# lionelblonde/sac-td3-cudagraphs-pytorch

Measured on NVIDIA B200. Metric: gradient updates/sec (batch 256, Hopper shapes), higher is better.
Workload: dtype f32

## Files before the change

### sac_td3_cudagraphs_pytorch_b200/csrc/api.cu

```cuda
#include <cstdarg>
#include <cstdio>
#include <cstdlib>
#include <cstring>

#include "common.cuh"

namespace b2rl {
cudaError_t launch_critic_fused(const b2rl_update_args_t&, cudaStream_t);
cudaError_t launch_actor_fused(const b2rl_update_args_t&, cudaStream_t);
cudaError_t launch_alpha(const b2rl_update_args_t&, float, cudaStream_t);
cudaError_t launch_alpha_adam(float*, uint64_t*, int, float, const b2rl_agent_hp_t*, float, float*, cudaStream_t);
cudaError_t launch_predict(const b2rl_update_args_t&, const float*, int, int, float, uint64_t, float*, cudaStream_t);
cudaError_t launch_wgrad(const b2rl_update_args_t&, int, int, const b2rl_adam_args_t*, cudaStream_t, int skip_vec = 0);
cudaError_t launch_adam(const b2rl_adam_args_t&, cudaStream_t);
cudaError_t launch_sumsq(const float*, int64_t, int64_t, int64_t, int64_t, int, float*, float*, cudaStream_t);
cudaError_t launch_bump(uint64_t*, int, int, cudaStream_t);
cudaError_t launch_gather(const float*, int64_t, int64_t, b2rl_rowfmt_t, int, int, const int64_t*, int64_t*, float*,
                          uint64_t, uint64_t*, int, int, int, cudaStream_t);
cudaError_t launch_extend(float*, int64_t, int64_t, b2rl_rowfmt_t, const float*, int, cudaStream_t);
cudaError_t launch_publish(const float*, int, float*, uint64_t*, uint64_t*, cudaStream_t);
cudaError_t launch_extend_dev(float*, int64_t, int64_t, b2rl_rowfmt_t, const float*, int, int, uint64_t*, cudaStream_t);
int max_in_dim_critic();
int max_in_dim_actor();
cudaError_t init_critic();
// ... 332 lines not shown
                      "wide_critic_scalars");
}
int b2rl_wide_actor_loss(const float* q0, const float* q1, const float* logp, const float* log_alpha, int32_t td3, int32_t M,
                         float* dzq0, float* dzq1, float* part, const b2rl_stack_t* stack, void* stream) {
  if (int rc = check_stack(stack, "wide_actor_loss")) return rc;
  if (!q0 || !dzq0 || !part || M < 1 || (!td3 && (!q1 || !dzq1 || !logp || !log_alpha)))
    return fail(B2RL_E_INVALID, "wide_actor_loss: bad arguments");
  return check_launch(b2rl::launch_wide_actor_loss(q0, q1, logp, log_alpha, td3, M, dzq0, dzq1, part, make_stk(stack), (cudaStream_t)stream), "wide_actor_loss");
}
int b2rl_wide_dqda(const float* dz1, const float* w1a, int32_t A, int32_t M, float* dqda, const b2rl_stack_t* stack, void* stream) {
  if (int rc = check_stack(stack, "wide_dqda")) return rc;
  if (!dz1 || !w1a || !dqda || A < 1 || A > 32 || M < 1) return fail(B2RL_E_INVALID, "wide_dqda: bad arguments");
  return check_launch(b2rl::launch_wide_dqda(dz1, w1a, A, M, dqda, make_stk(stack), (cudaStream_t)stream), "wide_dqda");
}
int b2rl_wide_actor_head_bwd(const float* dqda0, const float* dqda1, const float* save, const float* min_ac,
                             const float* max_ac, const float* log_alpha, int32_t td3, int32_t A, int32_t M, float* du,
                             float* part_du, const b2rl_stack_t* stack, void* stream) {
  if (int rc = check_stack(stack, "wide_actor_head_bwd")) return rc;
  if (!dqda0 || !save || !min_ac || !max_ac || !du || !part_du || A < 1 || A > 32 || M < 1 || (!td3 && !log_alpha))
    return fail(B2RL_E_INVALID, "wide_actor_head_bwd: bad arguments");
  return check_launch(b2rl::launch_wide_actor_head_bwd(dqda0, dqda1, save, min_ac, max_ac, log_alpha, td3, A, M, du, part_du,
                                                       make_stk(stack), (cudaStream_t)stream), "wide_actor_head_bwd");
}
int b2rl_wide_actor_scalars(const float* part_s, const float* part_du, int32_t P, int32_t M, int32_t out_dim, int32_t td3,
                            const float* log_alpha, float* G, int64_t off_b3, float* out, const b2rl_stack_t* stack, void* stream) {
  if (int rc = check_stack(stack, "wide_actor_scalars")) return rc;
  if (!part_s || !part_du || !G || !out || P < 1 || M < 1 || out_dim < 1 || out_dim > B2RL_MAX_OUT)
    return fail(B2RL_E_INVALID, "wide_actor_scalars: bad arguments");
  return check_launch(b2rl::launch_wide_actor_scalars(part_s, part_du, P, M, out_dim, td3, log_alpha, G, off_b3, out, make_stk(stack), (cudaStream_t)stream),
                      "wide_actor_scalars");
}
int b2rl_wide_alpha_grad(const float* logp2, int32_t M, float targ_ent, float* alpha_state, const b2rl_stack_t* stack, void* stream) {
  if (int rc = check_stack(stack, "wide_alpha_grad")) return rc;
  if (!logp2 || !alpha_state || M < 1) return fail(B2RL_E_INVALID, "wide_alpha_grad: bad arguments");
  return check_launch(b2rl::launch_wide_alpha_grad(logp2, M, targ_ent, alpha_state, make_stk(stack), (cudaStream_t)stream), "wide_alpha_grad");
}
int64_t b2rl_tc_wgrad_scratch_floats(int32_t MA, int32_t Bn, int32_t n_agents) {
  if (MA < 1 || Bn < 1 || n_agents < 0) return -1;
  const int64_t per_agent = (int64_t)b2rl::tc_wgrad_splits(Bn, MA, n_agents > 0) * ((MA + 127) / 128 * 128) * B2RL_HID;
  return per_agent * (n_agents > 0 ? n_agents : 1);
}
int b2rl_tc_wgrad(const float* A, int64_t lda, int32_t a_cols, int32_t MA, const float* Bm, int32_t Bn, float* C, float* Ct,
                  float* scratch, int32_t x3, uint64_t* bump, const b2rl_stack_t* stack, void* stream) {
  if (int rc = check_stack(stack, "tc_wgrad")) return rc;
  if (!A || !Bm || !C || !scratch || MA < 1 || a_cols < MA || lda < a_cols || (lda & 3) || Bn < 1)
    return fail(B2RL_E_INVALID, "tc_wgrad: bad arguments");
  if (!aligned16(A) || !aligned16(Bm) || !aligned16(C) || !aligned16(scratch)) return fail(B2RL_E_INVALID, "tc_wgrad: 16-byte aligned tensors");
  if (Ct && (MA & 3)) return fail(B2RL_E_INVALID, "tc_wgrad: the transposed copy needs MA % 4 == 0");
  return check_launch(b2rl::launch_tc_wgrad(A, lda, a_cols, MA, Bm, Bn, C, Ct, scratch, x3, (unsigned long long*)bump, make_stk(stack),
                                            stack != nullptr, (cudaStream_t)stream), "tc_wgrad");
}
int b2rl_wgrad(const b2rl_update_args_t* a, int32_t actor_step, int32_t bump_counter, int32_t skip_vectors, void* stream) {
  if (int rc = check_update(a, actor_step != 0)) return rc;
  if (bump_counter < -1 || bump_counter > 3) return fail(B2RL_E_INVALID, "wgrad: bad bump_counter");
  return check_launch(b2rl::launch_wgrad(*a, actor_step != 0, bump_counter, nullptr, (cudaStream_t)stream, skip_vectors != 0), "wgrad");
}

int b2rl_publish_logs(const float* out, int32_t n_agents, float* host_out, uint64_t* seq_dev, uint64_t* host_seq,
                      void* stream) {
  if (!out || !host_out || !seq_dev || !host_seq || n_agents < 1) return fail(B2RL_E_INVALID, "publish_logs: bad arguments");
  return check_launch(b2rl::launch_publish(out, n_agents, host_out, seq_dev, host_seq, (cudaStream_t)stream), "publish_logs");
}

static int check_opt(const b2rl_update_args_t* a, const b2rl_adam_args_t* o, int64_t begin, int64_t end, int counter) {
  if (!o) return B2RL_OK;
  if (o->n_seg < 1 || o->n_seg > B2RL_MAX_SEG) return fail(B2RL_E_INVALID, "opt: n_seg %d out of range", o->n_seg);
  if (o->lo)
    return fail(B2RL_E_INVALID, "opt: the fused optimizer does not keep a lo mirror current; use the three-launch form");
  if (a->agent_hp || o->agent_hp)
    return fail(B2RL_E_INVALID, "opt: the fused optimizer takes no per-agent hyperparameter table; use the three-launch form");
  const b2rl_seg_t& s0 = o->seg[0];
  if (!s0.do_adam || s0.clip || s0.grad_scale != 1.0f || s0.begin != begin || s0.end != end || s0.counter != counter)
    return fail(B2RL_E_INVALID, "opt: seg[0] must be an unclipped, unscaled Adam segment over the trained nets");
  for (int i = 1; i < o->n_seg; ++i) {
    const b2rl_seg_t& s = o->seg[i];
    if (s.do_adam || !s.do_polyak || s.begin < 0 || s.end < s.begin || (s.begin & 3) || (s.end & 3) || s.end > a->region_stride)
      return fail(B2RL_E_INVALID, "opt: extra segment %d must be a 4-float aligned Polyak-only span", i);
  }
  return B2RL_OK;
}

static int critic_update(const b2rl_update_args_t* a, int td3, const b2rl_adam_args_t* opt, void* stream) {
  if (int rc = check_update(a, false)) return rc;
  if (opt && a->new_rows) return fail(B2RL_E_INVALID, "new_rows is not supported by the fused-optimizer entry point");
  if (int rc = check_opt(a, opt, a->critic[0].begin, a->critic[1].end, B2RL_CTR_Q)) return rc;
  if ((a->hp.td3 != 0) != (td3 != 0)) return fail(B2RL_E_INVALID, "hp.td3 does not match the entry point");
  if (int rc = check_launch(b2rl::launch_critic_fused(*a, (cudaStream_t)stream), "critic_fused")) return rc;
  return check_launch(b2rl::launch_wgrad(*a, 0, B2RL_CTR_Q, opt, (cudaStream_t)stream), "critic wgrad");
}
int b2rl_critic_update_sac(const b2rl_update_args_t* a, void* stream) { return critic_update(a, 0, nullptr, stream); }
int b2rl_critic_update_td3(const b2rl_update_args_t* a, void* stream) { return critic_update(a, 1, nullptr, stream); }
int b2rl_critic_update_opt(const b2rl_update_args_t* a, const b2rl_adam_args_t* opt, void* stream) {
  if (!a || !opt) return fail(B2RL_E_INVALID, "null args");
  return critic_update(a, a->hp.td3 != 0, opt, stream);
}

static int actor_update(const b2rl_update_args_t* a, int td3, const b2rl_adam_args_t* opt, void* stream) {
  if (int rc = check_update(a, true)) return rc;
  if (int rc = check_opt(a, opt, a->actor.begin, a->actor.end, B2RL_CTR_PI)) return rc;
  if ((a->hp.td3 != 0) != (td3 != 0)) return fail(B2RL_E_INVALID, "hp.td3 does not match the entry point");
  if (int rc = check_launch(b2rl::launch_actor_fused(*a, (cudaStream_t)stream), "actor_fused")) return rc;
  return check_launch(b2rl::launch_wgrad(*a, 1, B2RL_CTR_PI, opt, (cudaStream_t)stream), "actor wgrad");
}
int b2rl_actor_update_sac(const b2rl_update_args_t* a, void* stream) { return actor_update(a, 0, nullptr, stream); }
int b2rl_actor_update_td3(const b2rl_update_args_t* a, void* stream) { return actor_update(a, 1, nullptr, stream); }
int b2rl_actor_update_opt(const b2rl_update_args_t* a, const b2rl_adam_args_t* opt, void* stream) {
  if (!a || !opt) return fail(B2RL_E_INVALID, "null args");
  return actor_update(a, a->hp.td3 != 0, opt, stream);
}

int b2rl_alpha_update(const b2rl_update_args_t* a, float log_alpha_lr, void* stream) {
  if (int rc = check_update(a, false)) return rc;
  if (a->hp.td3) return fail(B2RL_E_INVALID, "alpha_update is SAC-only");
  if (!(log_alpha_lr >= 0.f)) return fail(B2RL_E_INVALID, "log_alpha_lr must be >= 0");
  return check_launch(b2rl::launch_alpha(*a, log_alpha_lr, (cudaStream_t)stream), "alpha_update");
}

int b2rl_alpha_adam(float* log_alpha, uint64_t* counters, int32_t n_agents, float log_alpha_lr, float grad_scale,
                    float* out, void* stream) {
  if (!log_alpha || !counters || n_agents < 1 || !(log_alpha_lr > 0.f))
    return fail(B2RL_E_INVALID, "alpha_adam: bad arguments");
  return check_launch(b2rl::launch_alpha_adam(log_alpha, counters, n_agents, log_alpha_lr, nullptr, grad_scale, out,
                                              (cudaStream_t)stream),
                      "alpha_adam");
}

int b2rl_alpha_adam_hp(float* log_alpha, uint64_t* counters, int32_t n_agents, const b2rl_agent_hp_t* hp, float grad_scale,
                       float* out, void* stream) {
  if (!log_alpha || !counters || n_agents < 1 || !hp) return fail(B2RL_E_INVALID, "alpha_adam_hp: bad arguments");
  if (int rc = check_hp(hp, "alpha_adam_hp")) return rc;
  return check_launch(b2rl::launch_alpha_adam(log_alpha, counters, n_agents, 0.f, hp, grad_scale, out, (cudaStream_t)stream),
                      "alpha_adam_hp");
}

int b2rl_grad_sumsq(const float* arena, int64_t region_stride, int64_t arena_agent_stride, int64_t begin, int64_t end,
                    int32_t n_agents, float* sumsq, float* scratch, void* stream) {
  if (!arena || !sumsq || !scratch || begin < 0 || end < begin || n_agents < 1)
    return fail(B2RL_E_INVALID, "grad_sumsq: bad arguments");
  return check_launch(b2rl::launch_sumsq(arena, region_stride, arena_agent_stride, begin, end, n_agents, sumsq, scratch,
                                         (cudaStream_t)stream),
                      "grad_sumsq");
}

int b2rl_adam_polyak_multi(const b2rl_adam_args_t* a, void* stream) {
  if (!a || !a->arena || !a->counters) return fail(B2RL_E_INVALID, "adam: null args");
  if (a->n_seg < 1 || a->n_seg > B2RL_MAX_SEG) return fail(B2RL_E_INVALID, "adam: n_seg %d out of range", a->n_seg);
  if (a->n_agents < 1 || a->n_agents > 65535) return fail(B2RL_E_INVALID, "adam: bad n_agents");
  if (!aligned16(a->arena) || (a->region_stride & 3) || (a->arena_agent_stride & 3))
    return fail(B2RL_E_INVALID, "adam: arena must be 16-byte aligned, strides multiples of 4 floats");
  if (a->lo && (!aligned16(a->lo) || (a->lo_agent_stride & 3) || a->lo_agent_stride < 2 * a->region_stride))
    return fail(B2RL_E_INVALID, "adam: the lo mirror must be 16-byte aligned, its agent stride >= 2 regions and a multiple of 4 floats");
  if (a->n_shadow < 0 || a->n_shadow > 3) return fail(B2RL_E_INVALID, "adam: n_shadow %d out of range", a->n_shadow);
  if (int rc = check_hp(a->agent_hp, "adam")) return rc;
  for (int q = 0; q < a->n_shadow; ++q) {
    const int64_t src = a->shadow_src[q], dst = a->shadow_dst[q], n = (int64_t)B2RL_HID * B2RL_HID;
    if (src < 0 || dst < 0 || (src & 3) || (dst & 3) || src + n > a->region_stride || dst + n > a->region_stride ||
        (src < dst + n && dst < src + n))
      return fail(B2RL_E_INVALID, "adam: shadow pair %d must be two disjoint, 4-float aligned 256x256 spans of a region", q);
    for (int i = 0; i < a->n_seg; ++i) {
      const b2rl_seg_t& s = a->seg[i];
      const bool in_src = src >= s.begin && src + n <= s.end, in_dst = dst >= s.begin && dst + n <= s.end;
      const bool cut = (src < s.end && src + n > s.begin && !in_src) || (dst < s.end && dst + n > s.begin && !in_dst);
      if (cut || in_src != in_dst) return fail(B2RL_E_INVALID, "adam: segment %d splits shadow pair %d", i, q);
    }
  }
  for (int i = 0; i < a->n_seg; ++i) {
    const b2rl_seg_t& s = a->seg[i];
// ... 56 lines not shown
```

### sac_td3_cudagraphs_pytorch_b200/csrc/wgrad.cu

```cuda
#include "adam_math.cuh"

namespace b2rl {

constexpr int TM = 32, TN = 32;
constexpr int WT = 256, WW = WT / 32;

struct GemmJob {
  const float* A;
  const float* Bm;
  float* C;
  float* Ct;
  int lda, ldb, M;
};

struct OptCtx {
  int adam, polyak;
  AdamScalars k;
  float beta2, omb1, omb2, eps, pk;
  int64_t region;
};
static __device__ __noinline__ void opt_apply4(const OptCtx* ocp, float* gptr) {
  const OptCtx& oc = *ocp;
  float* P = gptr - 4 * oc.region;
  float4 p = *reinterpret_cast<const float4*>(P);
  float4 tg = make_float4(0.f, 0.f, 0.f, 0.f);
  if (oc.polyak) tg = *reinterpret_cast<const float4*>(P + oc.region);
  if (oc.adam) {
    const float4 g = *reinterpret_cast<const float4*>(gptr);
    float4 m = *reinterpret_cast<const float4*>(P + 2 * oc.region);
    float4 v = *reinterpret_cast<const float4*>(P + 3 * oc.region);
    adam_elem(p.x, g.x, m.x, v.x, oc.k, oc.beta2, oc.omb1, oc.omb2, oc.eps);
    adam_elem(p.y, g.y, m.y, v.y, oc.k, oc.beta2, oc.omb1, oc.omb2, oc.eps);
    adam_elem(p.z, g.z, m.z, v.z, oc.k, oc.beta2, oc.omb1, oc.omb2, oc.eps);
    adam_elem(p.w, g.w, m.w, v.w, oc.k, oc.beta2, oc.omb1, oc.omb2, oc.eps);
    *reinterpret_cast<float4*>(P) = p;
    *reinterpret_cast<float4*>(P + 2 * oc.region) = m;
    *reinterpret_cast<float4*>(P + 3 * oc.region) = v;
  }
  if (oc.polyak) {
    tg.x = polyak_elem(tg.x, p.x, oc.pk); tg.y = polyak_elem(tg.y, p.y, oc.pk);
    tg.z = polyak_elem(tg.z, p.z, oc.pk); tg.w = polyak_elem(tg.w, p.w, oc.pk);
    *reinterpret_cast<float4*>(P + oc.region) = tg;
  }
}
static __device__ __noinline__ void opt_apply1(const OptCtx* ocp, float* gptr) {
  const OptCtx& oc = *ocp;
  float* P = gptr - 4 * oc.region;
  float p = *P;
  float tg = oc.polyak ? P[oc.region] : 0.f;
  if (oc.adam) {
    float m = P[2 * oc.region], v = P[3 * oc.region];
    adam_elem(p, *gptr, m, v, oc.k, oc.beta2, oc.omb1, oc.omb2, oc.eps);
    *P = p; P[2 * oc.region] = m; P[3 * oc.region] = v;
  }
  if (oc.polyak) P[oc.region] = polyak_elem(tg, p, oc.pk);
}

constexpr int CHUNK = 32;
struct WgradSmem {
  union {
    float stage[WW][2][CHUNK][TM];
    float red[WW][TM][TN + 1];
  };
};

__device__ __forceinline__ void cp_async16(void* smem_dst, const void* gsrc, bool valid) {
  const unsigned d = (unsigned)__cvta_generic_to_shared(smem_dst);
  const int n = valid ? 16 : 0;
  asm volatile("cp.async.cg.shared.global [%0], [%1], 16, %2;" ::"r"(d), "l"(gsrc), "r"(n) : "memory");
}

template <typename Setup>
__device__ void gemm_tile(const GemmJob& J, int B, int m0, int n0, WgradSmem& S, const OptCtx* oc, Setup setup) {
  const int t = threadIdx.x, w = t >> 5, l = t & 31;
  const int mi = (l >> 2) * 4, ni = (l & 3) * 8;
  const int bs = (B + WW - 1) / WW;
  const int bA = min(B, w * bs), bB = min(B, bA + bs);
  float acc[4][8];
#pragma unroll
  for (int i = 0; i < 4; ++i)
#pragma unroll
    for (int j = 0; j < 8; ++j) acc[i][j] = 0.f;
  float(*As)[TM] = S.stage[w][0];
  float(*Bs)[TM] = S.stage[w][1];
  for (int b0 = bA; b0 < bB; b0 += CHUNK) {
    const int nb = min(CHUNK, bB - b0);
    for (int idx = l; idx < nb * 8; idx += 32) {
      const int row = idx >> 3, seg = (idx & 7) * 4;
      cp_async16(&As[row][seg], J.A + (size_t)(b0 + row) * J.lda + m0 + seg, m0 + seg + 3 < J.lda);
      cp_async16(&Bs[row][seg], J.Bm + (size_t)(b0 + row) * J.ldb + n0 + seg, true);
    }
    asm volatile("cp.async.commit_group;\n cp.async.wait_group 0;" ::: "memory");
    __syncwarp();
#pragma unroll 4
    for (int row = 0; row < nb; ++row) {
      const float4 a = *reinterpret_cast<const float4*>(&As[row][mi]);
      const float4 x0 = *reinterpret_cast<const float4*>(&Bs[row][ni]);
      const float4 x1 = *reinterpret_cast<const float4*>(&Bs[row][ni + 4]);
      const float av[4] = {a.x, a.y, a.z, a.w};
      const float xv[8] = {x0.x, x0.y, x0.z, x0.w, x1.x, x1.y, x1.z, x1.w};
#pragma unroll
      for (int i = 0; i < 4; ++i)
#pragma unroll
        for (int j = 0; j < 8; ++j) acc[i][j] = fmaf(av[i], xv[j], acc[i][j]);
    }
    __syncwarp();
  }
  setup();
  __syncthreads();
#pragma unroll
  for (int i = 0; i < 4; ++i)
#pragma unroll
    for (int j = 0; j < 8; ++j) S.red[w][mi + i][ni + j] = acc[i][j];
  __syncthreads();
  const int i = t >> 3, j0 = (t & 7) * 4;
  float s[4];
#pragma unroll
  for (int j = 0; j < 4; ++j) {
    float v = S.red[0][i][j0 + j];
#pragma unroll
    for (int ww = 1; ww < WW; ++ww) v += S.red[ww][i][j0 + j];
    s[j] = v;
  }
  if (m0 + i < J.M) {
    float* gp = J.C + (size_t)(m0 + i) * HID + n0 + j0;
    const float4 g4 = make_float4(s[0], s[1], s[2], s[3]);
    *reinterpret_cast<float4*>(gp) = g4;
    if (oc) opt_apply4(oc, gp);
  }
  if (J.Ct) {
    __syncthreads();
#pragma unroll
    for (int j = 0; j < 4; ++j) S.red[0][i][j0 + j] = s[j];
    __syncthreads();
    const int jj = t >> 3, i0 = (t & 7) * 4;
    if (m0 + i0 + 3 < J.M) {
      float* gp = J.Ct + (size_t)(n0 + jj) * J.M + m0 + i0;
      const float4 g4 = make_float4(S.red[0][i0][jj], S.red[0][i0 + 1][jj], S.red[0][i0 + 2][jj], S.red[0][i0 + 3][jj]);
      *reinterpret_cast<float4*>(gp) = g4;
      if (oc) opt_apply4(oc, gp);
    }
  }
}

constexpr int XTRA_CTAS = 16;

struct WgradArgs {
  b2rl_update_args_t u;
  int actor_step;
  int bump_counter;
  int has_opt;
  int work_ctas;
  int skip_vec;
  b2rl_adam_args_t opt;
};

__device__ __forceinline__ const b2rl_net_t& net_of(const WgradArgs& W, int n) {
  return W.actor_step ? W.u.actor : W.u.critic[n];
}

__host__ __device__ inline int tiles_of_net(const b2rl_net_t& n) {
  const int nt = HID / TN;
  return ((n.in_dim + TM - 1) / TM) * nt + (HID / TM) * nt + ((n.out_dim + TM - 1) / TM) * nt;
}
constexpr int VEC_CTAS = PART_VEC + 1;

static __device__ __noinline__ unsigned long long setup_and_ticket(const WgradArgs& W, int agent, uint64_t cnt, OptCtx& oc_s) {
  uint64_t* ctr = W.u.counters + (size_t)agent * 8;
  if (W.has_opt) {
    const b2rl_seg_t& s0 = W.opt.seg[0];
    OptCtx o;
    o.adam = s0.do_adam; o.polyak = s0.do_polyak;
    o.k = adam_scalars(s0.lr, W.opt.beta1, W.opt.beta2, (float)(cnt + 1ULL));
    adam_finish(o.k, W.opt.eps);
    o.beta2 = W.opt.beta2; o.omb1 = 1.0f - W.opt.beta1; o.omb2 = 1.0f - W.opt.beta2; o.eps = W.opt.eps;
    o.pk = W.opt.polyak; o.region = W.u.region_stride;
    oc_s = o;
  }
  if (W.bump_counter < 0) return 0ULL;
  __threadfence();
  return atomicAdd((unsigned long long*)&ctr[B2RL_CTR_TICKET], 1ULL + (cnt & 0ULL));
}
template <bool OPT>
__device__ __forceinline__ void ticket_finish(const WgradArgs& W, int agent, uint64_t cnt, unsigned long long ticket) {
  if (!OPT) return;
  if (threadIdx.x != 0 || W.bump_counter < 0 || ticket != (unsigned long long)gridDim.x - 1) return;
  uint64_t* ctr = W.u.counters + (size_t)agent * 8;
  ctr[W.bump_counter] = cnt + 1ULL;
  ctr[B2RL_CTR_TICKET] = 0;
}

template <bool OPT>
__global__ void __launch_bounds__(WT) wgrad_kernel(const __grid_constant__ WgradArgs W) {
  pdl_enter();
  extern __shared__ __align__(16) unsigned char wsm_raw[];
  WgradSmem& S = *reinterpret_cast<WgradSmem*>(wsm_raw);
  __shared__ OptCtx oc_s;
  const b2rl_update_args_t& A = W.u;
  const int agent = blockIdx.y, t = threadIdx.x;
  const int B = A.batch, nblk = row_blocks(B);
  const int n_nets = W.actor_step ? 1 : 2;
  float* arena = A.arena + (size_t)agent * A.arena_agent_stride;
  float* G = arena + 4 * A.region_stride;
  const float* rows = A.rows + (size_t)agent * A.rows_agent_stride;
  float* wsb = A.workspace + (size_t)agent * A.workspace_agent_stride;
  const int nt = HID / TN;
  const OptCtx* oc = OPT ? &oc_s : nullptr;
  const int cidx = W.bump_counter >= 0 ? W.bump_counter : (W.has_opt ? W.opt.seg[0].counter : 0);
  const uint64_t cnt = (OPT && t == 0) ? A.counters[(size_t)agent * 8 + cidx] : 0ULL;
  unsigned long long ticket = 0ULL;
  auto setup = [&]() { if (OPT && t == 0) ticket = setup_and_ticket(W, agent, cnt, oc_s); };

  int id = blockIdx.x;
  if (OPT && id >= W.work_ctas) {
    const int64_t stride = (int64_t)XTRA_CTAS * WT * 4;
    float* P = arena;
    float* T = arena + A.region_stride;
    for (int si = 1; si < W.opt.n_seg; ++si) {
      const b2rl_seg_t& sg = W.opt.seg[si];
      for (int64_t i = sg.begin + ((int64_t)(id - W.work_ctas) * WT + t) * 4; i < sg.end; i += stride) {
        const float4 p = *reinterpret_cast<const float4*>(P + i);
        float4 tg = *reinterpret_cast<const float4*>(T + i);
        tg.x = polyak_elem(tg.x, p.x, W.opt.polyak); tg.y = polyak_elem(tg.y, p.y, W.opt.polyak);
        tg.z = polyak_elem(tg.z, p.z, W.opt.polyak); tg.w = polyak_elem(tg.w, p.w, W.opt.polyak);
        *reinterpret_cast<float4*>(T + i) = tg;
      }
    }
    setup();
    ticket_finish<OPT>(W, agent, cnt, ticket);
    return;
  }
  for (int n = 0; n < n_nets; ++n) {
    const b2rl_net_t& net = net_of(W, n);
    const Workspace ws = ws_carve(wsb, B, n);
    const int t1 = ((net.in_dim + TM - 1) / TM) * nt, t2 = (HID / TM) * nt, t3 = ((net.out_dim + TM - 1) / TM) * nt;
    if (id < t1 + t2 + t3) {
      GemmJob J;
      if (id < t1) {
        J = {rows, ws.dz1, G + net.w1t, nullptr, A.fmt.row_stride, HID, net.in_dim};
      } else if (id < t1 + t2) {
        id -= t1;
        J = {ws.h1, ws.dz2, G + net.w2t, net.w2n >= 0 ? G + net.w2n : nullptr, HID, HID, HID};
      } else {
        id -= t1 + t2;
        J = {ws.dz3, ws.h2, G + net.w3, nullptr, MAX_OUT, HID, net.out_dim};
      }
      gemm_tile(J, B, (id / nt) * TM, (id % nt) * TN, S, oc, setup);
      ticket_finish<OPT>(W, agent, cnt, ticket);
      return;
    }
    id -= t1 + t2 + t3;
    if (id < VEC_CTAS) {
      if (W.skip_vec) return;
      setup();
      __syncthreads();
      if (id < PART_VEC) {
        if (net.layer_norm || (id % 3) == 0) {
          const int64_t off = id == 0 ? net.b1 : id == 1 ? net.g1 : id == 2 ? net.be1 : id == 3 ? net.b2 : id == 4 ? net.g2 : net.be2;
          const float* p = ws.part + (size_t)id * HID + t;
          float s = 0.f;
#pragma unroll 16
          for (int i = 0; i < nblk; ++i) s += p[(size_t)i * PART_LEN];
          G[off + t] = s;
          if (oc) opt_apply1(oc, G + off + t);
        }
      } else {
        if (t < net.out_dim) {
          float s = 0.f;
#pragma unroll 16
          for (int i = 0; i < nblk; ++i) s += ws.part[(size_t)i * PART_LEN + PART_DB3 + t];
          G[net.b3 + t] = s;
          if (oc) opt_apply1(oc, G + net.b3 + t);
        }
        if ((t >> 5) == 2 && n == n_nets - 1) {
          const int lane = t & 31;
          float* out = A.out + (size_t)agent * 8;
          float tot = 0.f, lp = 0.f;
          for (int m = 0; m < n_nets; ++m) {
            const float* pm = ws_carve(wsb, B, m).part;
            float s0 = 0.f, s1 = 0.f;
            for (int i = lane; i < nblk; i += 32) {
              s0 += pm[(size_t)i * PART_LEN + PART_SCAL];
              s1 += pm[(size_t)i * PART_LEN + PART_SCAL + 1];
            }
            tot += warp_sum(s0) / (float)B;
            lp += warp_sum(s1);
          }
          if (lane == 0) {
            if (W.actor_step) {
              out[B2RL_OUT_ACTOR_LOSS] = tot;
              out[B2RL_OUT_LOGPI_MEAN] = lp / (float)B;
              if (!A.hp.td3) out[B2RL_OUT_ALPHA] = expf(A.log_alpha[(size_t)agent * 5]);
            } else {
              out[B2RL_OUT_QF_LOSS] = tot;
            }
          }
        }
      }
      ticket_finish<OPT>(W, agent, cnt, ticket);
      return;
    }
    id -= VEC_CTAS;
  }
  if (!OPT) {
    if (id == 0 && t == 0 && W.bump_counter >= 0) A.counters[(size_t)agent * 8 + W.bump_counter] += 1ULL;
    if (id == 0 && !W.actor_step && A.new_rows) {
      uint64_t* ctr = A.counters + (size_t)agent * 8;
      const int64_t cursor = (int64_t)ctr[B2RL_CTR_CURSOR];
      const int rs = A.fmt.row_stride, chunks = rs >> 2;
      float* sto = const_cast<float*>(A.storage) + (size_t)agent * A.storage_agent_stride;
      for (int i = t; i < A.n_new * chunks; i += blockDim.x) {
        const int r = i / chunks, c4 = i - r * chunks;
        const int64_t d = (cursor + r) % A.capacity;
        st_stream4(sto + (size_t)d * rs + 4 * c4, ld_stream4(A.new_rows + (size_t)r * rs + 4 * c4));
      }
      __syncthreads();
      if (t == 0) {
        ctr[B2RL_CTR_CURSOR] = (uint64_t)((cursor + A.n_new) % A.capacity);
        const uint64_t size = ctr[B2RL_CTR_SIZE] + (uint64_t)A.n_new;
        ctr[B2RL_CTR_SIZE] = size < (uint64_t)A.capacity ? size : (uint64_t)A.capacity;
      }
    }
    return;
  }
  setup();
  ticket_finish<OPT>(W, agent, cnt, ticket);
}

cudaError_t init_wgrad() {
  cudaError_t e = cudaFuncSetAttribute(wgrad_kernel<false>, cudaFuncAttributeMaxDynamicSharedMemorySize, (int)sizeof(WgradSmem));
  if (e == cudaSuccess)
    e = cudaFuncSetAttribute(wgrad_kernel<true>, cudaFuncAttributeMaxDynamicSharedMemorySize, (int)sizeof(WgradSmem));
  return e;
}

cudaError_t launch_wgrad(const b2rl_update_args_t& a, int actor_step, int bump_counter, const b2rl_adam_args_t* opt,
                         cudaStream_t st, int skip_vec) {
  WgradArgs W;
  W.skip_vec = skip_vec;
  W.u = a;
  W.actor_step = actor_step;
  W.bump_counter = bump_counter;
  W.has_opt = opt != nullptr;
  if (opt) W.opt = *opt;
  int ctas = 0;
  const int n_nets = actor_step ? 1 : 2;
  for (int n = 0; n < n_nets; ++n) ctas += tiles_of_net(actor_step ? a.actor : a.critic[n]) + VEC_CTAS;
  W.work_ctas = ctas;
  if (opt && opt->n_seg > 1) ctas += XTRA_CTAS;
  if (!opt) ctas += 1;
  dim3 grid(ctas, a.n_agents);
  if (opt) return launch_k(wgrad_kernel<true>, grid, dim3(WT), -1, sizeof(WgradSmem), st, W);
  return launch_k(wgrad_kernel<false>, grid, dim3(WT), -1, sizeof(WgradSmem), st, W);
}

}
```

### sac_td3_cudagraphs_pytorch_b200/engine.py

```python
from __future__ import annotations

import ctypes as C
from typing import Optional

import numpy as np
import torch

from . import _lib as L
from .agents.agent import Agent
from .replay import Batch, ReplayBuffer
from .staging import StepStaging


class LearnerEngine:
    def __init__(self, agent: Agent, rb: Optional[ReplayBuffer] = None, batch_size: Optional[int] = None,
                 use_graphs: Optional[bool] = None, record_noise: bool = False, fused_opt: bool = False,
                 fused_sample: Optional[bool] = None):
        self.agent = agent
        self.rb = rb if rb is not None else agent.rb
        assert self.rb is not None and self.rb.storage is not None, "the replay buffer must hold data"
        self.B = int(batch_size or agent.hps.batch_size)
        self.use_graphs = bool(agent.hps.cudagraphs) if use_graphs is None else use_graphs
        self.fused_opt = bool(fused_opt)
        self.fused_sample = True if fused_sample is None else bool(fused_sample)
        dev = agent.device
        self.rows = torch.zeros(self.B, agent.fmt.row_stride, dtype=torch.float32, device=dev)
        self.idx = torch.zeros(self.B, dtype=torch.int64, device=dev)
        delay = int(agent.hps.actor_update_delay)
        mk = (lambda: torch.zeros(self.B, agent.ac_dim, device=dev)) if record_noise else (lambda: None)
        self.noise_q, self.noise_pi, self.noise_alpha = mk(), [mk() for _ in range(delay)], [mk() for _ in range(delay)]
        self.args_q = agent.update_args(self.rows, eps_out=self.noise_q,
                                        storage=self.rb.storage if self.fused_sample else None, idx_out=self.idx)
        self.args_pi = [agent.update_args(self.rows, eps_out=self.noise_pi[j], eps2_out=self.noise_alpha[j])
                        for j in range(delay)]
        self.graphs: dict[tuple, torch.cuda.CUDAGraph] = {}
        self._size_on_device = -1
        self._cursor_on_device = -1
        self.launches_per_variant: dict[tuple, int] = {}
        self._stage = StepStaging(dev, (), agent.fmt.row_stride, agent.ob_dim, agent.ac_dim)
        self.host_out = self._stage.host_outs[0]
        self._keep: list = []
        self._side_stream = torch.cuda.Stream(device=dev)

    def _enqueue(self, do_actor: bool, do_polyak: bool, args_q=None, before_last_adam=None) -> int:
        ag, rb = self.agent, self.rb
        args_q = args_q or self.args_q
        st = ag._stream()
        n = 0
        if not self.fused_sample:
            L.check(ag._lib.b2rl_replay_sample_gather(
                rb.storage.data_ptr(), 0, 0, rb.fmt, self.B, 1, None, self.idx.data_ptr(), self.rows.data_ptr(),
                C.c_uint64(ag.seed), ag.counters.data_ptr(), L.CTR_Q, 0, ag.agent_id, st), "replay_sample_gather")
            n += 1
        delay = int(ag.hps.actor_update_delay) if do_actor else 0
        extra = ag.polyak_segs(critics=False, actor=True) if (ag.td3 and do_polyak and delay == 0) else []
        fused = ag.fuses_opt(self.fused_opt)
        hook = None if fused else before_last_adam
        ag.enqueue_critic_step(args_q, extra_segs=extra, polyak=do_polyak, fused_opt=fused,
                               before_adam=hook if delay == 0 else None)
        n += 2 if fused else 3
        for j in range(delay):
            ag.enqueue_actor_step(self.args_pi[j], polyak=ag.td3 and do_polyak and j == delay - 1,
                                  fused_opt=fused,
                                  before_adam=hook if (j == delay - 1 and not ag.autotune) else None)
            n += (5 if ag.hps.clip_norm > 0 else (2 if fused else 3)) + (1 if ag.autotune else 0)
        return n

    def _polyak_due(self) -> bool:
        ag = self.agent
        return ag.td3 or ((ag.qnet_updates_so_far + 1) % ag.hps.crit_targ_update_freq == 0)

    def _sync_size(self) -> None:
        if self._size_on_device != len(self.rb):
            self._size_on_device = len(self.rb)
            self.agent.counters[L.CTR_SIZE] = self._size_on_device
        if self._cursor_on_device != self.rb._cursor:
            self._cursor_on_device = self.rb._cursor
            self.agent.counters[L.CTR_CURSOR] = self._cursor_on_device

    def host_rows(self, n: int, slot: Optional[int] = None) -> torch.Tensor:
        return self._stage.rows(n, slot)

    def host_obs(self, n: int, slot: Optional[int] = None) -> torch.Tensor:
        return self._stage.obs(n, slot)

    def wait_actions(self) -> "np.ndarray":
        return self._stage.actions()

    def step_async(self, i: int, n_new: int = 0, n_obs: int = 0, explore: bool = True) -> int:
        ag, rb = self.agent, self.rb
        assert self.use_graphs, "step() is the graph path"
        slot = self._stage.begin()
        do_actor = (i % (ag.hps.actor_update_delay + 1) == 0)
        key = (do_actor, self._polyak_due(), int(n_new), slot, int(n_obs), bool(explore))
        self._sync_size()
        g = self.graphs.get(key)
        if g is None:
            g = self._capture_step(key)
        g.replay()
        if n_new:
            rb._cursor = (rb._cursor + n_new) % rb.capacity
            rb._size = min(rb.capacity, rb._size + n_new)
            self._cursor_on_device, self._size_on_device = rb._cursor, rb._size
        ag.qnet_updates_so_far += 1
        if do_actor:
            ag.actor_updates_so_far += int(ag.hps.actor_update_delay)
        return self._stage.launched(n_obs, slot)

    def wait(self, ticket: int, as_numpy: bool = False):
        return self._stage.wait(ticket, as_numpy)

    def step(self, i: int, n_new: int = 0, n_obs: int = 0, explore: bool = True) -> torch.Tensor:
        return self.wait(self.step_async(i, n_new, n_obs, explore))

    def _capture_step(self, key) -> torch.cuda.CUDAGraph:
        ag, rb, stage = self.agent, self.rb, self._stage
        do_actor, do_polyak, n_new, slot, n_obs, explore = key
        new_rows = stage.rows(n_new, slot) if n_new else None
        if n_obs:
            obs = stage.obs(n_obs, slot)
            pa = L.UpdateArgs()
            pa.hp, pa.fmt, pa.actor = ag._hyper, ag.fmt, ag.layout.actor.c_struct()
            pa.arena, pa.region_stride, pa.agent_base = ag.arena.flat.data_ptr(), ag.layout.region, ag.agent_id
            pa.min_ac, pa.max_ac, pa.counters = ag.min_ac.data_ptr(), ag.max_ac.data_ptr(), ag.counters.data_ptr()
            self._keep.append(pa)
        g = torch.cuda.CUDAGraph()
        torch.cuda.synchronize(ag.device)
        with torch.cuda.graph(g):
            n = 0
            if n_obs:
                std = float(ag.hps.actor_noise_std) if ag.td3 else 0.0
                L.check(ag._lib.b2rl_actor_predict(C.byref(pa), obs.data_ptr(), n_obs, int(explore), std,
                                                   C.c_uint64(2 ** 64 - 1), stage.device_actions(n_obs).data_ptr(), ag._stream()),
                        "actor_predict")
                stage.publish_actions(ag._lib, n_obs, slot, ag._stream())
                n += 2
            args_q = None
            if n_new and self.fused_sample and not ag.fuses_opt(self.fused_opt):
                args_q = ag.update_args(self.rows, eps_out=self.noise_q, storage=rb.storage, idx_out=self.idx,
                                        new_rows=new_rows, n_new=n_new)
                self._keep.append(args_q)
            elif n_new:
                L.check(ag._lib.b2rl_replay_extend_dev(rb.storage.data_ptr(), rb.capacity, rb.fmt,
                                                       new_rows.data_ptr(), n_new, ag.counters.data_ptr(),
                                                       ag._stream()), "replay_extend_dev")
                n += 1
            joined = []

            def publish():
                stage.publish_logs(ag._lib, ag.out, slot, ag._stream())

            def fork_publish():
                main, ev = torch.cuda.current_stream(ag.device), torch.cuda.Event()
                ev.record(main)
                self._side_stream.wait_event(ev)
                with torch.cuda.stream(self._side_stream):
                    publish()
                    done = torch.cuda.Event()
                    done.record(self._side_stream)
                joined.append(done)

            n += self._enqueue(do_actor, do_polyak, args_q, before_last_adam=fork_publish)
            if joined:
                torch.cuda.current_stream(ag.device).wait_event(joined[0])
            else:
                publish()
            n += 1
        self.launches_per_variant[key] = n
        self.graphs[key] = g
        return g

    def iteration(self, i: int) -> None:
        ag = self.agent
        do_actor = (i % (ag.hps.actor_update_delay + 1) == 0)
        key = (do_actor, self._polyak_due())
        self._sync_size()
        if not self.use_graphs:
            self.launches_per_variant[key] = self._enqueue(*key)
        else:
            g = self.graphs.get(key)
            if g is None:
                g = self._capture(key)
            g.replay()
        ag.qnet_updates_so_far += 1
        if do_actor:
            ag.actor_updates_so_far += int(ag.hps.actor_update_delay)

    def _capture(self, key) -> torch.cuda.CUDAGraph:
        g = torch.cuda.CUDAGraph()
        torch.cuda.synchronize(self.agent.device)
        with torch.cuda.graph(g):
            self.launches_per_variant[key] = self._enqueue(*key)
        self.graphs[key] = g
        return g

    def launches(self, i: int) -> int:
        key = (i % (self.agent.hps.actor_update_delay + 1) == 0, self._polyak_due())
        return self.launches_per_variant.get(key, 0)

    def logs(self) -> dict[str, torch.Tensor]:
        ag, o = self.agent, self.agent.out
        d = {"loss/qf_loss": o[L.OUT_QF_LOSS], "loss/actor_loss": o[L.OUT_ACTOR_LOSS]}
        if not ag.td3:
            d["vitals/alpha"] = o[L.OUT_ALPHA]
            if ag.autotune:
                d["loss/alpha_loss"] = o[L.OUT_ALPHA_LOSS]
        return d

    def last_batch(self) -> Batch:
        return Batch(self.rows, self.agent.fmt, self.idx)
```

Measured before the change: 16280.

## Enable fused optimizer by default and fold replay writes, prefetch, Polyak into wgrad

Makes the fused Adam/Polyak optimizer path the default when gradient clipping is off. The replay-buffer write moves into a dedicated CTA of the fused wgrad kernel, removing a separate extend launch. Optimizer state is prefetched into L1 before the GEMM tile runs, and the transposed-gradient optimizer update reuses staged shared-memory results instead of reloading state. The extra Polyak CTA count is now sized from the segment lengths, with two float4 loads per iteration. The new path adds shared-memory staging and extra synchronisation, and risks ordering problems if replay writes overlap with sampling.

```diff
diff --git a/sac_td3_cudagraphs_pytorch_b200/csrc/api.cu b/sac_td3_cudagraphs_pytorch_b200/csrc/api.cu
--- a/sac_td3_cudagraphs_pytorch_b200/csrc/api.cu
+++ b/sac_td3_cudagraphs_pytorch_b200/csrc/api.cu
@@ -438,7 +438,6 @@
 
 static int critic_update(const b2rl_update_args_t* a, int td3, const b2rl_adam_args_t* opt, void* stream) {
   if (int rc = check_update(a, false)) return rc;
-  if (opt && a->new_rows) return fail(B2RL_E_INVALID, "new_rows is not supported by the fused-optimizer entry point");
   if (int rc = check_opt(a, opt, a->critic[0].begin, a->critic[1].end, B2RL_CTR_Q)) return rc;
   if ((a->hp.td3 != 0) != (td3 != 0)) return fail(B2RL_E_INVALID, "hp.td3 does not match the entry point");
   if (int rc = check_launch(b2rl::launch_critic_fused(*a, (cudaStream_t)stream), "critic_fused")) return rc;
diff --git a/sac_td3_cudagraphs_pytorch_b200/csrc/wgrad.cu b/sac_td3_cudagraphs_pytorch_b200/csrc/wgrad.cu
--- a/sac_td3_cudagraphs_pytorch_b200/csrc/wgrad.cu
+++ b/sac_td3_cudagraphs_pytorch_b200/csrc/wgrad.cu
@@ -1,3 +1,5 @@
+#include <algorithm>
+
 #include "adam_math.cuh"
 
 namespace b2rl {
@@ -14,45 +16,56 @@
 };
 
 struct OptCtx {
-  int adam, polyak;
+  int polyak;
   AdamScalars k;
   float beta2, omb1, omb2, eps, pk;
   int64_t region;
 };
-static __device__ __noinline__ void opt_apply4(const OptCtx* ocp, float* gptr) {
+__device__ __forceinline__ void prefetch_l1(const float* p) { asm volatile("prefetch.global.L1 [%0];" ::"l"(p)); }
+__device__ __forceinline__ void opt_prefetch(const float* gptr, int64_t region, bool polyak) {
+  const float* P = gptr - 4 * region;
+  prefetch_l1(P);
+  if (polyak) prefetch_l1(P + region);
+  prefetch_l1(P + 2 * region);
+  prefetch_l1(P + 3 * region);
+}
+static __device__ __noinline__ void opt_apply4(const OptCtx* ocp, float* gptr, float4 g, float* stage) {
   const OptCtx& oc = *ocp;
   float* P = gptr - 4 * oc.region;
   float4 p = *reinterpret_cast<const float4*>(P);
   float4 tg = make_float4(0.f, 0.f, 0.f, 0.f);
   if (oc.polyak) tg = *reinterpret_cast<const float4*>(P + oc.region);
-  if (oc.adam) {
-    const float4 g = *reinterpret_cast<const float4*>(gptr);
-    float4 m = *reinterpret_cast<const float4*>(P + 2 * oc.region);
-    float4 v = *reinterpret_cast<const float4*>(P + 3 * oc.region);
-    adam_elem(p.x, g.x, m.x, v.x, oc.k, oc.beta2, oc.omb1, oc.omb2, oc.eps);
-    adam_elem(p.y, g.y, m.y, v.y, oc.k, oc.beta2, oc.omb1, oc.omb2, oc.eps);
-    adam_elem(p.z, g.z, m.z, v.z, oc.k, oc.beta2, oc.omb1, oc.omb2, oc.eps);
-    adam_elem(p.w, g.w, m.w, v.w, oc.k, oc.beta2, oc.omb1, oc.omb2, oc.eps);
-    *reinterpret_cast<float4*>(P) = p;
-    *reinterpret_cast<float4*>(P + 2 * oc.region) = m;
-    *reinterpret_cast<float4*>(P + 3 * oc.region) = v;
-  }
+  float4 m = *reinterpret_cast<const float4*>(P + 2 * oc.region);
+  float4 v = *reinterpret_cast<const float4*>(P + 3 * oc.region);
+  adam_elem(p.x, g.x, m.x, v.x, oc.k, oc.beta2, oc.omb1, oc.omb2, oc.eps);
+  adam_elem(p.y, g.y, m.y, v.y, oc.k, oc.beta2, oc.omb1, oc.omb2, oc.eps);
+  adam_elem(p.z, g.z, m.z, v.z, oc.k, oc.beta2, oc.omb1, oc.omb2, oc.eps);
+  adam_elem(p.w, g.w, m.w, v.w, oc.k, oc.beta2, oc.omb1, oc.omb2, oc.eps);
+  *reinterpret_cast<float4*>(P) = p;
+  *reinterpret_cast<float4*>(P + 2 * oc.region) = m;
+  *reinterpret_cast<float4*>(P + 3 * oc.region) = v;
   if (oc.polyak) {
     tg.x = polyak_elem(tg.x, p.x, oc.pk); tg.y = polyak_elem(tg.y, p.y, oc.pk);
     tg.z = polyak_elem(tg.z, p.z, oc.pk); tg.w = polyak_elem(tg.w, p.w, oc.pk);
     *reinterpret_cast<float4*>(P + oc.region) = tg;
   }
-}
-static __device__ __noinline__ void opt_apply1(const OptCtx* ocp, float* gptr) {
+  if (stage) {
+    constexpr int SL = TM * (TN + 1);
+    const float4 o[4] = {p, m, v, tg};
+#pragma unroll
+    for (int q = 0; q < 4; ++q) {
+      stage[q * SL] = o[q].x; stage[q * SL + 1] = o[q].y; stage[q * SL + 2] = o[q].z; stage[q * SL + 3] = o[q].w;
+    }
+  }
+}
+static __device__ __noinline__ void opt_apply1(const OptCtx* ocp, float* gptr, float g) {
   const OptCtx& oc = *ocp;
   float* P = gptr - 4 * oc.region;
-  float p = *P;
-  float tg = oc.polyak ? P[oc.region] : 0.f;
-  if (oc.adam) {
-    float m = P[2 * oc.region], v = P[3 * oc.region];
-    adam_elem(p, *gptr, m, v, oc.k, oc.beta2, oc.omb1, oc.omb2, oc.eps);
-    *P = p; P[2 * oc.region] = m; P[3 * oc.region] = v;
-  }
+  float p = P[0];
+  const float tg = oc.polyak ? P[oc.region] : 0.f;
+  float m = P[2 * oc.region], v = P[3 * oc.region];
+  adam_elem(p, g, m, v, oc.k, oc.beta2, oc.omb1, oc.omb2, oc.eps);
+  P[0] = p; P[2 * oc.region] = m; P[3 * oc.region] = v;
   if (oc.polyak) P[oc.region] = polyak_elem(tg, p, oc.pk);
 }
 
@@ -70,12 +83,17 @@
   asm volatile("cp.async.cg.shared.global [%0], [%1], 16, %2;" ::"r"(d), "l"(gsrc), "r"(n) : "memory");
 }
 
-template <typename Setup>
-__device__ void gemm_tile(const GemmJob& J, int B, int m0, int n0, WgradSmem& S, const OptCtx* oc, Setup setup) {
+template <bool OPT, typename Setup>
+__device__ void gemm_tile(const GemmJob& J, int B, int m0, int n0, WgradSmem& S, const OptCtx* oc, int64_t region, bool polyak,
+                          Setup setup) {
   const int t = threadIdx.x, w = t >> 5, l = t & 31;
   const int mi = (l >> 2) * 4, ni = (l & 3) * 8;
   const int bs = (B + WW - 1) / WW;
   const int bA = min(B, w * bs), bB = min(B, bA + bs);
+  const int i = t >> 3, j0 = (t & 7) * 4;
+  float* gp = J.C + (size_t)(m0 + i) * HID + n0 + j0;
+  const bool row_ok = m0 + i < J.M;
+  if (OPT && row_ok) opt_prefetch(gp, region, polyak);
   float acc[4][8];
 #pragma unroll
   for (int i = 0; i < 4; ++i)
@@ -113,7 +131,6 @@
 #pragma unroll
     for (int j = 0; j < 8; ++j) S.red[w][mi + i][ni + j] = acc[i][j];
   __syncthreads();
-  const int i = t >> 3, j0 = (t & 7) * 4;
   float s[4];
 #pragma unroll
   for (int j = 0; j < 4; ++j) {
@@ -122,28 +139,48 @@
     for (int ww = 1; ww < WW; ++ww) v += S.red[ww][i][j0 + j];
     s[j] = v;
   }
-  if (m0 + i < J.M) {
-    float* gp = J.C + (size_t)(m0 + i) * HID + n0 + j0;
-    const float4 g4 = make_float4(s[0], s[1], s[2], s[3]);
-    *reinterpret_cast<float4*>(gp) = g4;
-    if (oc) opt_apply4(oc, gp);
-  }
+  const float4 g4 = make_float4(s[0], s[1], s[2], s[3]);
+  if (row_ok) *reinterpret_cast<float4*>(gp) = g4;
+  if (J.Ct) __syncthreads();
+  if (OPT && row_ok) opt_apply4(oc, gp, g4, J.Ct ? &S.red[1][i][j0] : nullptr);
   if (J.Ct) {
-    __syncthreads();
 #pragma unroll
     for (int j = 0; j < 4; ++j) S.red[0][i][j0 + j] = s[j];
     __syncthreads();
     const int jj = t >> 3, i0 = (t & 7) * 4;
     if (m0 + i0 + 3 < J.M) {
-      float* gp = J.Ct + (size_t)(n0 + jj) * J.M + m0 + i0;
-      const float4 g4 = make_float4(S.red[0][i0][jj], S.red[0][i0 + 1][jj], S.red[0][i0 + 2][jj], S.red[0][i0 + 3][jj]);
-      *reinterpret_cast<float4*>(gp) = g4;
-      if (oc) opt_apply4(oc, gp);
-    }
-  }
-}
-
-constexpr int XTRA_CTAS = 16;
+      auto col = [&](int q) { return make_float4(S.red[q][i0][jj], S.red[q][i0 + 1][jj], S.red[q][i0 + 2][jj], S.red[q][i0 + 3][jj]); };
+      float* gt = J.Ct + (size_t)(n0 + jj) * J.M + m0 + i0;
+      *reinterpret_cast<float4*>(gt) = col(0);
+      if (OPT) {
+        float* P = gt - 4 * region;
+        *reinterpret_cast<float4*>(P) = col(1);
+        *reinterpret_cast<float4*>(P + 2 * region) = col(2);
+        *reinterpret_cast<float4*>(P + 3 * region) = col(3);
+        if (polyak) *reinterpret_cast<float4*>(P + region) = col(4);
+      }
+    }
+  }
+}
+
+__device__ void replay_write(const b2rl_update_args_t& A, int agent) {
+  const int t = threadIdx.x;
+  uint64_t* ctr = A.counters + (size_t)agent * 8;
+  const int64_t cursor = (int64_t)ctr[B2RL_CTR_CURSOR];
+  const int rs = A.fmt.row_stride, chunks = rs >> 2;
+  float* sto = const_cast<float*>(A.storage) + (size_t)agent * A.storage_agent_stride;
+  for (int i = t; i < A.n_new * chunks; i += blockDim.x) {
+    const int r = i / chunks, c4 = i - r * chunks;
+    const int64_t d = (cursor + r) % A.capacity;
+    st_stream4(sto + (size_t)d * rs + 4 * c4, ld_stream4(A.new_rows + (size_t)r * rs + 4 * c4));
+  }
+  __syncthreads();
+  if (t == 0) {
+    ctr[B2RL_CTR_CURSOR] = (uint64_t)((cursor + A.n_new) % A.capacity);
+    const uint64_t size = ctr[B2RL_CTR_SIZE] + (uint64_t)A.n_new;
+    ctr[B2RL_CTR_SIZE] = size < (uint64_t)A.capacity ? size : (uint64_t)A.capacity;
+  }
+}
 
 struct WgradArgs {
   b2rl_update_args_t u;
@@ -151,6 +188,7 @@
   int bump_counter;
   int has_opt;
   int work_ctas;
+  int write_cta;
   int skip_vec;
   b2rl_adam_args_t opt;
 };
@@ -170,7 +208,7 @@
   if (W.has_opt) {
     const b2rl_seg_t& s0 = W.opt.seg[0];
     OptCtx o;
-    o.adam = s0.do_adam; o.polyak = s0.do_polyak;
+    o.polyak = s0.do_polyak;
     o.k = adam_scalars(s0.lr, W.opt.beta1, W.opt.beta2, (float)(cnt + 1ULL));
     adam_finish(o.k, W.opt.eps);
     o.beta2 = W.opt.beta2; o.omb1 = 1.0f - W.opt.beta1; o.omb2 = 1.0f - W.opt.beta2; o.eps = W.opt.eps;
@@ -211,19 +249,33 @@
   unsigned long long ticket = 0ULL;
   auto setup = [&]() { if (OPT && t == 0) ticket = setup_and_ticket(W, agent, cnt, oc_s); };
 
+  const int64_t region = A.region_stride;
+  const bool polyak = OPT && W.opt.seg[0].do_polyak;
   int id = blockIdx.x;
   if (OPT && id >= W.work_ctas) {
-    const int64_t stride = (int64_t)XTRA_CTAS * WT * 4;
-    float* P = arena;
-    float* T = arena + A.region_stride;
-    for (int si = 1; si < W.opt.n_seg; ++si) {
-      const b2rl_seg_t& sg = W.opt.seg[si];
-      for (int64_t i = sg.begin + ((int64_t)(id - W.work_ctas) * WT + t) * 4; i < sg.end; i += stride) {
-        const float4 p = *reinterpret_cast<const float4*>(P + i);
-        float4 tg = *reinterpret_cast<const float4*>(T + i);
+    id -= W.work_ctas;
+    if (id < W.write_cta) {
+      replay_write(A, agent);
+    } else {
+      id -= W.write_cta;
+      const int64_t step = (int64_t)(gridDim.x - W.work_ctas - W.write_cta) * WT * 4;
+      float* P = arena;
+      float* T = arena + region;
+      auto lerp4 = [&](float4 tg, const float4& p) {
         tg.x = polyak_elem(tg.x, p.x, W.opt.polyak); tg.y = polyak_elem(tg.y, p.y, W.opt.polyak);
         tg.z = polyak_elem(tg.z, p.z, W.opt.polyak); tg.w = polyak_elem(tg.w, p.w, W.opt.polyak);
-        *reinterpret_cast<float4*>(T + i) = tg;
+        return tg;
+      };
+      for (int si = 1; si < W.opt.n_seg; ++si) {
+        const b2rl_seg_t& sg = W.opt.seg[si];
+        for (int64_t i = sg.begin + ((int64_t)id * WT + t) * 4; i < sg.end; i += 2 * step) {
+          const bool two = i + step < sg.end;
+          const float4 p0 = *reinterpret_cast<const float4*>(P + i), t0 = *reinterpret_cast<const float4*>(T + i);
+          float4 p1 = p0, t1 = t0;
+          if (two) p1 = *reinterpret_cast<const float4*>(P + i + step), t1 = *reinterpret_cast<const float4*>(T + i + step);
+          *reinterpret_cast<float4*>(T + i) = lerp4(t0, p0);
+          if (two) *reinterpret_cast<float4*>(T + i + step) = lerp4(t1, p1);
+        }
       }
     }
     setup();
@@ -245,32 +297,35 @@
         id -= t1 + t2;
         J = {ws.dz3, ws.h2, G + net.w3, nullptr, MAX_OUT, HID, net.out_dim};
       }
-      gemm_tile(J, B, (id / nt) * TM, (id % nt) * TN, S, oc, setup);
+      gemm_tile<OPT>(J, B, (id / nt) * TM, (id % nt) * TN, S, oc, region, polyak, setup);
       ticket_finish<OPT>(W, agent, cnt, ticket);
       return;
     }
     id -= t1 + t2 + t3;
     if (id < VEC_CTAS) {
       if (W.skip_vec) return;
+      const bool col = id < PART_VEC ? (net.layer_norm || (id % 3) == 0) : t < net.out_dim;
+      const int64_t off = id == 0 ? net.b1 : id == 1 ? net.g1 : id == 2 ? net.be1 : id == 3 ? net.b2 : id == 4 ? net.g2
+                        : id == 5 ? net.be2 : net.b3;
+      if (OPT && col) opt_prefetch(G + off + t, region, polyak);
       setup();
       __syncthreads();
       if (id < PART_VEC) {
-        if (net.layer_norm || (id % 3) == 0) {
-          const int64_t off = id == 0 ? net.b1 : id == 1 ? net.g1 : id == 2 ? net.be1 : id == 3 ? net.b2 : id == 4 ? net.g2 : net.be2;
+        if (col) {
           const float* p = ws.part + (size_t)id * HID + t;
           float s = 0.f;
 #pragma unroll 16
           for (int i = 0; i < nblk; ++i) s += p[(size_t)i * PART_LEN];
           G[off + t] = s;
-          if (oc) opt_apply1(oc, G + off + t);
+          if (OPT) opt_apply1(oc, G + off + t, s);
         }
       } else {
-        if (t < net.out_dim) {
+        if (col) {
           float s = 0.f;
 #pragma unroll 16
           for (int i = 0; i < nblk; ++i) s += ws.part[(size_t)i * PART_LEN + PART_DB3 + t];
-          G[net.b3 + t] = s;
-          if (oc) opt_apply1(oc, G + net.b3 + t);
+          G[off + t] = s;
+          if (OPT) opt_apply1(oc, G + off + t, s);
         }
         if ((t >> 5) == 2 && n == n_nets - 1) {
           const int lane = t & 31;
@@ -302,29 +357,9 @@
     }
     id -= VEC_CTAS;
   }
-  if (!OPT) {
-    if (id == 0 && t == 0 && W.bump_counter >= 0) A.counters[(size_t)agent * 8 + W.bump_counter] += 1ULL;
-    if (id == 0 && !W.actor_step && A.new_rows) {
-      uint64_t* ctr = A.counters + (size_t)agent * 8;
-      const int64_t cursor = (int64_t)ctr[B2RL_CTR_CURSOR];
-      const int rs = A.fmt.row_stride, chunks = rs >> 2;
-      float* sto = const_cast<float*>(A.storage) + (size_t)agent * A.storage_agent_stride;
-      for (int i = t; i < A.n_new * chunks; i += blockDim.x) {
-        const int r = i / chunks, c4 = i - r * chunks;
-        const int64_t d = (cursor + r) % A.capacity;
-        st_stream4(sto + (size_t)d * rs + 4 * c4, ld_stream4(A.new_rows + (size_t)r * rs + 4 * c4));
-      }
-      __syncthreads();
-      if (t == 0) {
-        ctr[B2RL_CTR_CURSOR] = (uint64_t)((cursor + A.n_new) % A.capacity);
-        const uint64_t size = ctr[B2RL_CTR_SIZE] + (uint64_t)A.n_new;
-        ctr[B2RL_CTR_SIZE] = size < (uint64_t)A.capacity ? size : (uint64_t)A.capacity;
-      }
-    }
-    return;
-  }
-  setup();
-  ticket_finish<OPT>(W, agent, cnt, ticket);
+  if (OPT || id != 0) return;
+  if (t == 0 && W.bump_counter >= 0) A.counters[(size_t)agent * 8 + W.bump_counter] += 1ULL;
+  if (!W.actor_step && A.new_rows) replay_write(A, agent);
 }
 
 cudaError_t init_wgrad() {
@@ -347,7 +382,13 @@
   const int n_nets = actor_step ? 1 : 2;
   for (int n = 0; n < n_nets; ++n) ctas += tiles_of_net(actor_step ? a.actor : a.critic[n]) + VEC_CTAS;
   W.work_ctas = ctas;
-  if (opt && opt->n_seg > 1) ctas += XTRA_CTAS;
+  W.write_cta = opt && !actor_step && a.new_rows ? 1 : 0;
+  ctas += W.write_cta;
+  if (opt && opt->n_seg > 1) {
+    int64_t n = 0;
+    for (int i = 1; i < opt->n_seg; ++i) n += opt->seg[i].end - opt->seg[i].begin;
+    ctas += (int)std::min<int64_t>(std::max<int64_t>((n + WT * 8 - 1) / (WT * 8), 1), 148);
+  }
   if (!opt) ctas += 1;
   dim3 grid(ctas, a.n_agents);
   if (opt) return launch_k(wgrad_kernel<true>, grid, dim3(WT), -1, sizeof(WgradSmem), st, W);
diff --git a/sac_td3_cudagraphs_pytorch_b200/engine.py b/sac_td3_cudagraphs_pytorch_b200/engine.py
--- a/sac_td3_cudagraphs_pytorch_b200/engine.py
+++ b/sac_td3_cudagraphs_pytorch_b200/engine.py
@@ -14,14 +14,14 @@
 
 class LearnerEngine:
     def __init__(self, agent: Agent, rb: Optional[ReplayBuffer] = None, batch_size: Optional[int] = None,
-                 use_graphs: Optional[bool] = None, record_noise: bool = False, fused_opt: bool = False,
+                 use_graphs: Optional[bool] = None, record_noise: bool = False, fused_opt: Optional[bool] = None,
                  fused_sample: Optional[bool] = None):
         self.agent = agent
         self.rb = rb if rb is not None else agent.rb
         assert self.rb is not None and self.rb.storage is not None, "the replay buffer must hold data"
         self.B = int(batch_size or agent.hps.batch_size)
         self.use_graphs = bool(agent.hps.cudagraphs) if use_graphs is None else use_graphs
-        self.fused_opt = bool(fused_opt)
+        self.fused_opt = (agent.hps.clip_norm <= 0) if fused_opt is None else bool(fused_opt)
         self.fused_sample = True if fused_sample is None else bool(fused_sample)
         dev = agent.device
         self.rows = torch.zeros(self.B, agent.fmt.row_stride, dtype=torch.float32, device=dev)
@@ -136,7 +136,7 @@
                 stage.publish_actions(ag._lib, n_obs, slot, ag._stream())
                 n += 2
             args_q = None
-            if n_new and self.fused_sample and not ag.fuses_opt(self.fused_opt):
+            if n_new and self.fused_sample:
                 args_q = ag.update_args(self.rows, eps_out=self.noise_q, storage=rb.storage, idx_out=self.idx,
                                         new_rows=new_rows, n_new=n_new)
                 self._keep.append(args_q)
```

Result: slower. 16090 (median of 6 runs) (-1.2%).
